# pkusys/Auncel

Hardware: AMD Instinct MI355X
Metric: queries/sec @ recall@10>=0.95, SIFT-10M d=128 IVF4096, 1/2/4/8 GPU (higher is better)
Workload: dtype u8

## Files before the change

### auncel_amd/csrc/ivf_plan.hip

```cpp
#include "ivf_dev.h"

#include <stdlib.h>

namespace amdivf {

__device__ __forceinline__ void plan_begin(const PlanArgs& a, uint32_t tid, uint32_t nthreads) {
    if (tid < 16 && a.history) a.history[tid] = a.counters[tid];
    if (tid == 0 && a.first_plan) {
        a.bytes[0] = 0.0;
        a.acc64[0] = a.acc64[1] = 0ull;
        if (a.min_bytes) a.min_bytes[0] = 0.0;
        if (a.min_bytes_thr) a.min_bytes_thr[0] = 0.0;
    }
    if (a.first_plan && a.round_unfinished)
        for (uint32_t r = tid; r < PLAN_MAX_ROUNDS * 8; r += nthreads) a.round_unfinished[r] = 0;
}
__device__ __forceinline__ void plan_counts_query(const PlanArgs& a, uint32_t i, uint32_t lane) {
    const bool have = i < a.nq;
    uint32_t cnt = 0, pad = 0, more = 0;
    unsigned long long need = 0;
    const unsigned long long ra = a.row_align - 1;
    if (have && !a.done[i]) {
        const uint32_t stage = a.stage[i];
        unsigned long long target = (unsigned long long)stage + a.round_len;
        const unsigned long long np = a.my_nprobe ? a.my_nprobe[a.id_offset + i] : 0ull;
        if (a.tune) {
            const unsigned long long safe = (unsigned long long)((float)(stage + 1) * a.multipler);
            const unsigned long long g = (unsigned long long)((double)stage * a.grow);
            target = safe > g ? safe : g;
            const unsigned long long inc = stage == 0 ? a.first_round : a.min_inc;
            if (target < (unsigned long long)stage + inc) target = (unsigned long long)stage + inc;
        }
        if (np != 0) target = np > (unsigned long long)stage + 1 ? np : (unsigned long long)stage + 1;
        bool last = false;
        if (a.budget_ms) {
            target = (unsigned long long)stage + a.first_round;
            if (stage > 0) {
                const float per = a.elapsed_ms / (float)stage, room = 0.95f * a.budget_ms[a.id_offset + i] - a.elapsed_ms;
                const float fit = room > 0.f ? floorf(room / fmaxf(per, 1e-9f)) : 0.f;
                const unsigned long long cap = stage > a.first_round ? stage : a.first_round;
                unsigned long long len = fit >= (float)a.total_nprobe ? a.total_nprobe : (unsigned long long)fit;
                if (len < 1) len = 1;
                last = len <= cap;
                target = (unsigned long long)stage + (last ? len : cap);
            }
        }
        if (target > a.total_nprobe) target = a.total_nprobe;
        if (a.run_dis && target > stage) {
            const float* dq = a.run_dis + (size_t)i * a.key_stride;
            const int64_t* ka = a.keys + (size_t)i * a.key_stride;
            while (target < a.total_nprobe && dq[target - 1] == dq[target] && ka[target] >= 0) target++;
        }
        if (a.limit && lane == 0) a.limit[i] = last ? (uint32_t)target : a.total_nprobe;
        if (target <= stage) target = stage + 1 < a.total_nprobe ? stage + 1 : a.total_nprobe;
        cnt = (uint32_t)(target - stage);
        const bool ends = target >= a.total_nprobe || last || (a.tune && np != 0);
        more = ends ? 0u : 1u;
        const int64_t* kq = a.keys + (size_t)i * a.key_stride + stage;
        for (uint32_t p = lane; p < cnt; p += 64) {
            const int64_t key = kq[p];
            if (key >= 0 && (unsigned long long)key < a.nlist) {
                const unsigned long long sz = a.list_off[key + 1] - a.list_off[key], psz = (sz + ra) & ~ra;
                need += psz;
                pad += (uint32_t)(psz - sz);
            }
        }
        for (int off = 32; off; off >>= 1) {
            need += __shfl_xor(need, off);
            pad += __shfl_xor(pad, off);
        }
    }
    if (have && lane == 0) {
        a.cnt[i] = cnt;
        a.need[i] = need;
        a.pad[i] = pad | (more << 31);
    }
}
__global__ __launch_bounds__(256) void plan_counts_kernel(PlanArgs a) {
    for (uint32_t l = blockIdx.x * 256 + threadIdx.x; l < 8 * a.nlist; l += gridDim.x * 256) a.xcount[l] = 0;
    if (blockIdx.x == 0) plan_begin(a, threadIdx.x, 256);
    plan_counts_query(a, blockIdx.x * 4 + (threadIdx.x >> 6), threadIdx.x & 63);
}

template <int N> __device__ __forceinline__ void block_scan_1024_n(const uint32_t (&v)[N], uint32_t (&excl)[N], uint32_t (&total)[N],
                                                                    uint32_t (*s_wave)[N]) {
    const int lane = threadIdx.x & 63, w = threadIdx.x >> 6, nw = (int)(blockDim.x >> 6);
    uint32_t incl[N];
#pragma unroll
    for (int k = 0; k < N; k++) incl[k] = v[k];
    for (int off = 1; off < 64; off <<= 1) {
#pragma unroll
        for (int k = 0; k < N; k++) {
            const uint32_t o = (uint32_t)__shfl_up((int)incl[k], off);
            if (lane >= off) incl[k] += o;
        }
    }
    if (lane == 63) {
#pragma unroll
        for (int k = 0; k < N; k++) s_wave[w][k] = incl[k];
    }
    __syncthreads();
    if (w == 0) {
#pragma unroll
        for (int k = 0; k < N; k++) {
            const uint32_t x = lane < nw ? s_wave[lane][k] : 0u;
            uint32_t inc = x;
            for (int off = 1; off < 16; off <<= 1) {
                const uint32_t o = (uint32_t)__shfl_up((int)inc, off);
                if (lane >= off) inc += o;
            }
            if (lane < nw) s_wave[lane][k] = inc - x;
            if (lane == nw - 1) s_wave[16][k] = inc;
        }
    }
    __syncthreads();
#pragma unroll
    for (int k = 0; k < N; k++) {
        excl[k] = s_wave[w][k] + incl[k] - v[k];
        total[k] = s_wave[16][k];
    }
    __syncthreads();
}

__device__ __forceinline__ void plan_prefix_body(const PlanArgs& a) {
    __shared__ uint32_t cut;
    const uint32_t t = threadIdx.x;
    if (t == 0) cut = 0xffffffffu;
    const uint32_t nt = blockDim.x;
    const uint32_t per = (a.nq + nt - 1) / nt, q0 = t * per < a.nq ? t * per : a.nq, q1 = q0 + per < a.nq ? q0 + per : a.nq;
    unsigned long long my_need = 0;
    uint32_t my_cnt = 0, my_act = 0;
    for (uint32_t i = q0; i < q1; i++) {
        const uint32_t c = a.cnt[i];
        my_cnt += c;
        my_act += c ? 1u : 0u;
        my_need += a.need[i];
    }
    unsigned long long tot_need;
    uint32_t ecnt, eact;
    unsigned long long eneed;
    {
        __shared__ uint32_t s_w4[17][4];
        const uint32_t v4[4] = {(uint32_t)(my_need & 0xfffffu), (uint32_t)(my_need >> 20), my_cnt, my_act};
        uint32_t e4[4], t4[4];
        block_scan_1024_n<4>(v4, e4, t4, s_w4);
        eneed = (unsigned long long)e4[0] + ((unsigned long long)e4[1] << 20);
        tot_need = (unsigned long long)t4[0] + ((unsigned long long)t4[1] << 20);
        ecnt = e4[2];
        eact = e4[3];
    }
    for (uint32_t i = q0; i < q1; i++) {
        const uint32_t c = a.cnt[i];
        const unsigned long long nd = a.need[i];
        const bool fits = (eneed + nd <= a.dist_budget && ecnt + c <= a.seg_cap) || eact == 0;
        if (c && !fits) atomicMin(&cut, i);
        a.seg_begin[i] = ecnt;
        a.dist_base[i] = eneed;
        if (c) a.qsel[eact] = i;
        eneed += nd;
        ecnt += c;
        eact += c ? 1u : 0u;
    }
    __syncthreads();
    uint32_t nact = 0, nseg = 0, nmore = 0, ndef = 0;
    unsigned long long ndist = 0;
    __shared__ uint32_t s_nact, s_nseg, s_more, s_def;
    __shared__ unsigned long long s_ndist;
    if (t == 0) {
        s_nact = 0;
        s_nseg = 0;
        s_more = 0;
        s_def = 0;
        s_ndist = 0;
    }
    __syncthreads();
    for (uint32_t i = t; i < a.nq; i += nt) {
        uint32_t c = a.cnt[i];
        const uint32_t pm = a.pad[i], pad = pm & 0x7fffffffu;
        if (pm >> 31) a.pad[i] = pad;
        if (i >= cut && c) {
            a.cnt[i] = c = 0;
            ndef++;
        }
        if (c) {
            nact++;
            nseg += c;
            ndist += a.need[i] - pad;
            nmore += pm >> 31;
        }
    }
    atomicAdd(&s_nact, nact);
    atomicAdd(&s_nseg, nseg);
    atomicAdd(&s_more, nmore);
    atomicAdd(&s_def, ndef);
    atomicAdd(&s_ndist, ndist);
    __syncthreads();
    if (t == 0) {
        a.counters[0] = s_nact;
        a.counters[1] = s_nseg;
        if (a.cl_cursor)
            for (int x = 0; x < 8; x++) a.cl_cursor[32 * x] = 0;
        a.counters[10] = s_more + s_def;
        a.counters[11] = s_def;
        a.counters[7] = (uint32_t)(s_ndist >> 20);
        a.counters[12] = (uint32_t)((tot_need + (1u << 20) - 1) >> 20);
        a.bytes[0] += (double)s_ndist * (double)a.d * 4.0;
        if (a.min_bytes) a.min_bytes[0] += a.dense_round ? (double)s_ndist * 4.0 : (double)s_ndist / 8.0;
        if (a.min_bytes_thr && !a.dense_round) a.min_bytes_thr[0] += (double)s_ndist / 8.0;
    }
}
__global__ __launch_bounds__(1024) void plan_prefix_kernel(PlanArgs a) { plan_prefix_body(a); }

__device__ __forceinline__ void plan_segments_query(const PlanArgs& a, uint32_t i, uint32_t c, uint32_t lane) {
    const uint32_t stage = a.stage[i];
    const uint32_t xcc = xcc_id();
    const int64_t* kq = a.keys + (size_t)i * a.key_stride + stage;
    unsigned long long cur = a.dist_base[i];
    const unsigned long long ra = a.row_align - 1;
    const uint32_t sb = a.seg_begin[i];
    for (uint32_t p0 = 0; p0 < c; p0 += 64) {
        const uint32_t p = p0 + lane;
        int64_t key = -1;
        unsigned long long psz = 0;
        if (p < c) {
            key = kq[p];
            if (key >= 0 && (unsigned long long)key < a.nlist) {
                const unsigned long long sz = a.list_off[key + 1] - a.list_off[key];
                if (sz) {
                    a.seg_slot[sb + p] = (xcc << 28) | xcd_local_add(&a.xcount[xcc * a.nlist + (uint32_t)key], 1u);
                    psz = (sz + ra) & ~ra;
                }
            }
        }
        unsigned long long incl = psz;
        for (int off = 1; off < 64; off <<= 1) {
            const unsigned long long o = __shfl_up(incl, off);
            if ((int)lane >= off) incl += o;
        }
        if (p < c) {
            a.seg_list[sb + p] = (int32_t)key;
            a.seg_off[sb + p] = cur + incl - psz;
        }
        cur += __shfl(incl, 63);
    }
}
__global__ __launch_bounds__(256) void plan_segments_kernel(PlanArgs a) {
    const uint32_t i = blockIdx.x * 4 + (threadIdx.x >> 6);
    const uint32_t c = i < a.nq ? a.cnt[i] : 0u;
    if (c) plan_segments_query(a, i, c, threadIdx.x & 63);
}


__device__ __forceinline__ void plan_lists_body(const PlanArgs& a) {
    __shared__ uint32_t s_w[17][6];
    const uint32_t t = threadIdx.x;
    auto values = [&](uint32_t l, uint32_t c, uint32_t (&v)[6]) {
#pragma unroll
        for (int k = 0; k < 6; k++) v[k] = 0;
        if (!c) return;
        const unsigned long long sz = a.list_off[l + 1] - a.list_off[l];
        v[0] = c;
        v[1] = (c + SCAN_RQ - 1) / SCAN_RQ;
        if (a.mfma_chunk) {
            v[5] = ((c + a.mfma_qblock - 1) / a.mfma_qblock) * (uint32_t)((sz + a.mfma_chunk - 1) / a.mfma_chunk);
            return;
        }
        const uint32_t full = c / a.qblock, rem = c % a.qblock;
        if (full) {
            const uint32_t qg = scan_shape_of(a.qblock);
            const uint32_t tv = scan_tile_vecs(qg);
            v[2 + scan_qg_class(qg)] = full * (uint32_t)((sz + tv - 1) / tv);
        }
        if (rem) {
            const uint32_t qg = scan_shape_of(rem);
            const uint32_t tv = scan_tile_vecs(qg);
            v[2 + scan_qg_class(qg)] += (uint32_t)((sz + tv - 1) / tv);
        }
    };
    auto book = [&](uint32_t l, uint32_t c, unsigned long long& slots, unsigned long long& useful) {
        if (!c) return;
        const unsigned long long sz = a.list_off[l + 1] - a.list_off[l];
        useful += (unsigned long long)c * sz;
        if (a.mfma_chunk) {
            const unsigned long long nvb = (sz + a.mfma_chunk - 1) / a.mfma_chunk, lastv = sz - (nvb - 1) * a.mfma_chunk;
            const unsigned long long vsum = (nvb - 1) * (((unsigned long long)a.mfma_chunk + 63) / 64 * 64) + (lastv + 63) / 64 * 64;
            const unsigned long long nqb = (c + a.mfma_qblock - 1) / a.mfma_qblock, lastq = c - (nqb - 1) * a.mfma_qblock;
            const unsigned long long qsum = (nqb - 1) * (((unsigned long long)a.mfma_qblock + MFMA_QBLOCK - 1) / MFMA_QBLOCK * MFMA_QBLOCK) +
                                            (lastq + MFMA_QBLOCK - 1) / MFMA_QBLOCK * MFMA_QBLOCK;
            slots += qsum * vsum;
            return;
        }
        const uint32_t full = c / a.qblock, rem = c % a.qblock;
        if (full) {
            const uint32_t tv = scan_tile_vecs(scan_shape_of(a.qblock));
            slots += (unsigned long long)full * ((a.qblock + SCAN_RQ - 1) / SCAN_RQ * SCAN_RQ) * ((sz + tv - 1) / tv) * tv;
        }
        if (rem) {
            const uint32_t tv = scan_tile_vecs(scan_shape_of(rem));
            slots += (unsigned long long)((rem + SCAN_RQ - 1) / SCAN_RQ * SCAN_RQ) * ((sz + tv - 1) / tv) * tv;
        }
    };
    const uint32_t nt = blockDim.x;
    const uint32_t per = (a.nlist + nt - 1) / nt, l0 = t * per < a.nlist ? t * per : a.nlist, l1 = l0 + per < a.nlist ? l0 + per : a.nlist;
    uint32_t mine[6] = {0, 0, 0, 0, 0, 0};
    double list_bytes = 0;
    unsigned long long my_slots = 0, my_useful = 0;
    for (uint32_t l = l0; l < l1; l++) {
        uint32_t c = 0;
#pragma unroll
        for (uint32_t x = 0; x < 8; x++) {
            const uint32_t cx = a.xcount[x * a.nlist + l];
            a.xcount[x * a.nlist + l] = c;
            c += cx;
        }
        a.lcount[l] = c;
        book(l, c, my_slots, my_useful);
        uint32_t v[6];
        values(l, c, v);
#pragma unroll
        for (int k = 0; k < 6; k++) mine[k] += v[k];
        if (v[0]) list_bytes += (double)(a.list_off[l + 1] - a.list_off[l]) * (double)a.row_bytes;
    }
    for (int off = 32; off; off >>= 1) {
        my_slots += __shfl_xor(my_slots, off);
        my_useful += __shfl_xor(my_useful, off);
    }
    if ((t & 63) == 0 && my_slots) {
        atomicAdd(&a.acc64[0], my_slots);
        atomicAdd(&a.acc64[1], my_useful);
    }
    if (a.min_bytes && list_bytes > 0) atomicAdd(a.min_bytes, list_bytes);
    if (a.min_bytes_thr && !a.dense_round && list_bytes > 0) atomicAdd(a.min_bytes_thr, list_bytes);
    uint32_t ex[6], tot[6];
    block_scan_1024_n<6>(mine, ex, tot, s_w);
    for (uint32_t l = l0; l < l1; l++) {
        uint32_t v[6];
        values(l, a.lcount[l], v);
        a.lstart[l] = ex[0];
        a.gbase[l] = ex[1];
        a.ibase[0 * a.nlist + l] = ex[2];
        a.ibase[1 * a.nlist + l] = ex[3];
        a.ibase[2 * a.nlist + l] = ex[4];
        a.ibase[3 * a.nlist + l] = ex[5];
#pragma unroll
        for (int k = 0; k < 6; k++) ex[k] += v[k];
    }
    if (t == 0) {
        const bool over = (unsigned long long)tot[2] + tot[3] + tot[4] + tot[5] > (unsigned long long)a.item_cap;
        if (over) {
            atomicMax(a.error, ERR_ITEM_OVERFLOW);
            tot[2] = tot[3] = tot[4] = tot[5] = 0;
        }
        a.counters[2] = tot[0];
        a.counters[3] = tot[1];
        a.counters[4] = tot[2];
        a.counters[5] = tot[3];
        a.counters[8] = tot[4];
        a.counters[9] = tot[5];
    }
}
__global__ __launch_bounds__(1024) void plan_lists_kernel(PlanArgs a) { plan_lists_body(a); }

__device__ __forceinline__ void plan_scatter_query(const PlanArgs& a, uint32_t i, uint32_t lane) {
    if (i >= a.nq) return;
    const uint32_t c = a.cnt[i];
    if (!c) return;
    const uint32_t sb = a.seg_begin[i];
    for (uint32_t p = lane; p < c; p += 64) {
        const int32_t key = a.seg_list[sb + p];
        if (key < 0 || (uint32_t)key >= a.nlist) continue;
        if (a.list_off[key + 1] == a.list_off[key]) continue;
        const uint32_t ss = a.seg_slot[sb + p];
        const uint32_t pos = a.lstart[key] + a.xcount[(ss >> 28) * a.nlist + (uint32_t)key] + (ss & 0x0fffffffu);
        a.pair_query[pos] = a.slot_base + i;
        a.pair_out[pos] = a.seg_off[sb + p];
    }
}

__device__ inline void items_of_list(const PlanArgs& a, uint32_t l, uint32_t c) {
    const uint32_t p0 = a.lstart[l], g0 = a.gbase[l];
    for (uint32_t o = 0, g = 0; o < c; o += SCAN_RQ, g++) {
        a.group_p0[g0 + g] = p0 + o;
        a.group_cnt[g0 + g] = c - o < (uint32_t)SCAN_RQ ? c - o : (uint32_t)SCAN_RQ;
    }
    const uint32_t n1 = a.counters[4], n2 = a.counters[5], n4 = a.counters[8];
    uint32_t cur[4] = {a.ibase[l], n1 + a.ibase[a.nlist + l], n1 + n2 + a.ibase[2 * a.nlist + l],
                       n1 + n2 + n4 + a.ibase[3 * a.nlist + l]};
    const uint32_t sz = (uint32_t)(a.list_off[l + 1] - a.list_off[l]);
    const uint64_t vb0 = a.list_off[l];
    const uint64_t lb0 = a.lane_block_off ? a.lane_block_off[l] : 0ull;
    if (a.mfma_chunk) {
        uint32_t ni = cur[3];
        const uint64_t b0 = a.block_off[l];
        const uint32_t nvb = (sz + a.mfma_chunk - 1) / a.mfma_chunk, nqb = (c + a.mfma_qblock - 1) / a.mfma_qblock;
        for (uint32_t o = 0; o < nvb * nqb; o++) {
            const uint32_t vb = (a.item_order ? o % nvb : o / nqb) * a.mfma_chunk, qb = (a.item_order ? o / nvb : o % nqb) * a.mfma_qblock;
            {
                ScanItem it;
                it.vec_base = b0 + vb / MFMA_BLOCK;
                it.nvec = sz - vb < a.mfma_chunk ? sz - vb : a.mfma_chunk;
                it.vec_off = vb;
                it.pair_begin = p0 + qb;
                it.npair = c - qb < a.mfma_qblock ? c - qb : a.mfma_qblock;
                it.qg = 0;
                it.qgroup = (uint32_t)(vb0 + vb);
                if (ni < a.item_cap) a.items[ni] = it;
                ni++;
            }
        }
        return;
    }
    for (uint32_t qb = 0; qb < c; qb += a.qblock) {
        const uint32_t nq_blk = c - qb < a.qblock ? c - qb : a.qblock;
        const uint32_t qg = scan_shape_of(nq_blk);
        const uint32_t tv = scan_tile_vecs(qg);
        uint32_t& ni = cur[scan_qg_class(qg)];
        for (uint32_t vb = 0; vb < sz; vb += tv) {
            ScanItem it;
            it.vec_base = scan_vec_base(vb0 + vb, lb0, vb);
            it.nvec = sz - vb < tv ? sz - vb : tv;
            it.vec_off = vb;
            it.pair_begin = p0 + qb;
            it.npair = nq_blk;
            it.qg = qg;
            it.qgroup = g0 + qb / SCAN_RQ;
            if (ni < a.item_cap) a.items[ni] = it;
            ni++;
        }
    }
}


__device__ __forceinline__ void plan_items_lists(const PlanArgs& a, uint32_t l) {
    const uint32_t c = l < a.nlist ? a.lcount[l] : 0u;
    if (c) items_of_list(a, l, c);
}

__device__ inline void items_of_list_wave(const PlanArgs& a, uint32_t l, uint32_t c, uint32_t lane) {
    const uint32_t p0 = a.lstart[l], g0 = a.gbase[l];
    for (uint32_t g = lane; g * SCAN_RQ < c; g += 64) {
        const uint32_t o = g * SCAN_RQ;
        a.group_p0[g0 + g] = p0 + o;
        a.group_cnt[g0 + g] = c - o < (uint32_t)SCAN_RQ ? c - o : (uint32_t)SCAN_RQ;
    }
    const uint32_t n1 = a.counters[4], n2 = a.counters[5], n4 = a.counters[8];
    const uint32_t cur[4] = {a.ibase[l], n1 + a.ibase[a.nlist + l], n1 + n2 + a.ibase[2 * a.nlist + l],
                             n1 + n2 + n4 + a.ibase[3 * a.nlist + l]};
    const uint32_t sz = (uint32_t)(a.list_off[l + 1] - a.list_off[l]);
    const uint64_t vb0 = a.list_off[l];
    const uint64_t lb0 = a.lane_block_off ? a.lane_block_off[l] : 0ull;
    if (a.mfma_chunk) {
        const uint64_t b0 = a.block_off[l];
        const uint32_t nvb = (sz + a.mfma_chunk - 1) / a.mfma_chunk, nqb = (c + a.mfma_qblock - 1) / a.mfma_qblock;
        for (uint32_t o = lane; o < nvb * nqb; o += 64) {
            const uint32_t vb = (a.item_order ? o % nvb : o / nqb) * a.mfma_chunk, qb = (a.item_order ? o / nvb : o % nqb) * a.mfma_qblock;
            ScanItem it;
            it.vec_base = b0 + vb / MFMA_BLOCK;
            it.nvec = sz - vb < a.mfma_chunk ? sz - vb : a.mfma_chunk;
            it.vec_off = vb;
            it.pair_begin = p0 + qb;
            it.npair = c - qb < a.mfma_qblock ? c - qb : a.mfma_qblock;
            it.qg = 0;
            it.qgroup = (uint32_t)(vb0 + vb);
            if (cur[3] + o < a.item_cap) a.items[cur[3] + o] = it;
        }
        return;
    }
    const uint32_t full = c / a.qblock, rem = c % a.qblock;
    const uint32_t qg_f = scan_shape_of(a.qblock), tv_f = scan_tile_vecs(qg_f), nt_f = (sz + tv_f - 1) / tv_f;
    const int cls_f = scan_qg_class(qg_f);
    for (uint32_t o = lane; o < full * nt_f; o += 64) {
        const uint32_t qb = (o / nt_f) * a.qblock, vb = (o % nt_f) * tv_f;
        ScanItem it;
        it.vec_base = scan_vec_base(vb0 + vb, lb0, vb);
        it.nvec = sz - vb < tv_f ? sz - vb : tv_f;
        it.vec_off = vb;
        it.pair_begin = p0 + qb;
        it.npair = a.qblock;
        it.qg = qg_f;
        it.qgroup = g0 + qb / SCAN_RQ;
        if (cur[cls_f] + o < a.item_cap) a.items[cur[cls_f] + o] = it;
    }
    if (rem) {
        const uint32_t qg_r = scan_shape_of(rem), tv_r = scan_tile_vecs(qg_r), nt_r = (sz + tv_r - 1) / tv_r;
        const int cls_r = scan_qg_class(qg_r);
        const uint32_t base = cur[cls_r] + (cls_r == cls_f ? full * nt_f : 0u), qb = full * a.qblock;
        for (uint32_t o = lane; o < nt_r; o += 64) {
            const uint32_t vb = o * tv_r;
            ScanItem it;
            it.vec_base = scan_vec_base(vb0 + vb, lb0, vb);
            it.nvec = sz - vb < tv_r ? sz - vb : tv_r;
            it.vec_off = vb;
            it.pair_begin = p0 + qb;
            it.npair = rem;
            it.qg = qg_r;
            it.qgroup = g0 + qb / SCAN_RQ;
            if (base + o < a.item_cap) a.items[base + o] = it;
        }
    }
}

__global__ __launch_bounds__(256) void plan_scatter_items_kernel(PlanArgs a, uint32_t gq) {
    if (blockIdx.x < gq) {
        plan_scatter_query(a, blockIdx.x * 4 + (threadIdx.x >> 6), threadIdx.x & 63);
        return;
    }
    const uint32_t l = (blockIdx.x - gq) * 4 + (threadIdx.x >> 6);
    const uint32_t c = l < a.nlist ? a.lcount[l] : 0u;
    if (c) items_of_list_wave(a, l, c, threadIdx.x & 63);
}

constexpr uint32_t PLAN_SMALL_NQ = 32;
__global__ __launch_bounds__(1024) void plan_small_kernel(PlanArgs a) {
    const uint32_t tid = threadIdx.x, lane = tid & 63, wave = tid >> 6;
    for (uint32_t l = tid; l < 8 * a.nlist; l += 1024) a.xcount[l] = 0;
    plan_begin(a, tid, 1024);
    __syncthreads();
    for (uint32_t i = wave; i < a.nq; i += 16) plan_counts_query(a, i, lane);
    __syncthreads();
    plan_prefix_body(a);
    __syncthreads();
    for (uint32_t i = wave; i < a.nq; i += 16) {
        const uint32_t c = a.cnt[i];
        if (c) plan_segments_query(a, i, c, lane);
    }
    __syncthreads();
    plan_lists_body(a);
    __syncthreads();
    for (uint32_t i = wave; i < a.nq; i += 16) plan_scatter_query(a, i, lane);
    for (uint32_t l0 = 0; l0 < a.nlist; l0 += 1024) plan_items_lists(a, l0 + tid);
}

__global__ __launch_bounds__(64) void plan_one_kernel(PlanArgs a) {
    const uint32_t lane = threadIdx.x;
    plan_begin(a, lane, 64);
    __syncthreads();
    plan_counts_query(a, 0, lane);
    __syncthreads();
    const uint32_t c = a.cnt[0];
    const unsigned long long nd = a.need[0];
    const uint32_t pm = a.pad[0], pad = pm & 0x7fffffffu;
    const unsigned long long ndist = c ? nd - pad : 0ull;
    if (lane == 0) {
        if (pm >> 31) a.pad[0] = pad;
        a.seg_begin[0] = 0;
        a.dist_base[0] = 0;
        if (c) a.qsel[0] = 0;
        a.counters[0] = c ? 1u : 0u;
        a.counters[1] = c;
        a.counters[10] = c ? pm >> 31 : 0u;
        a.counters[11] = 0;
        a.counters[7] = (uint32_t)(ndist >> 20);
        a.counters[12] = (uint32_t)((nd + (1u << 20) - 1) >> 20);
        a.bytes[0] += (double)ndist * (double)a.d * 4.0;
        if (a.min_bytes) a.min_bytes[0] += a.dense_round ? (double)ndist * 4.0 : (double)ndist / 8.0;
        if (a.min_bytes_thr && !a.dense_round) a.min_bytes_thr[0] += (double)ndist / 8.0;
    }
    const uint32_t stage = a.stage[0];
    const int64_t* kq = a.keys + stage;
    const unsigned long long ra = a.row_align - 1;
    const unsigned long long lt = lane == 0 ? 0ull : (~0ull >> (64 - lane));
    unsigned long long cur = 0, slots = 0, useful = 0;
    uint32_t np = 0, ni = 0;
    double list_bytes = 0;
    const uint32_t tv1 = scan_tile_vecs(1);
    for (uint32_t p0 = 0; p0 < c; p0 += 64) {
        const uint32_t p = p0 + lane;
        int64_t key = -1;
        uint32_t sz = 0;
        if (p < c) {
            key = kq[p];
            if (key >= 0 && (unsigned long long)key < a.nlist) sz = (uint32_t)(a.list_off[key + 1] - a.list_off[key]);
        }
        const bool valid = sz != 0;
        const unsigned long long psz = valid ? ((unsigned long long)sz + ra) & ~ra : 0ull;
        unsigned long long incl = psz;
        for (int off = 1; off < 64; off <<= 1) {
            const unsigned long long o = __shfl_up(incl, off);
            if ((int)lane >= off) incl += o;
        }
        const unsigned long long my_off = cur + incl - psz;
        if (p < c) {
            a.seg_list[p] = (int32_t)key;
            a.seg_off[p] = my_off;
        }
        cur += __shfl(incl, 63);
        const unsigned long long vm = __ballot(valid);
        const uint32_t pidx = np + (uint32_t)__builtin_popcountll(vm & lt);
        const uint32_t tile = a.mfma_chunk ? a.mfma_chunk : tv1;
        const uint32_t n_it = valid ? (sz + tile - 1) / tile : 0u;
        uint32_t iincl = n_it;
        for (int off = 1; off < 64; off <<= 1) {
            const uint32_t o = (uint32_t)__shfl_up((int)iincl, off);
            if ((int)lane >= off) iincl += o;
        }
        const uint32_t ibase = ni + iincl - n_it;
        if (valid) {
            a.pair_query[pidx] = a.slot_base;
            a.pair_out[pidx] = my_off;
            a.group_p0[pidx] = pidx;
            a.group_cnt[pidx] = 1;
            const uint64_t vb0 = a.list_off[key];
            const uint64_t b0 = a.mfma_chunk ? a.block_off[key] : 0ull;
            for (uint32_t o = 0; o < n_it; o++) {
                const uint32_t vb = o * tile;
                ScanItem it;
                it.vec_base = a.mfma_chunk ? b0 + vb / MFMA_BLOCK : scan_vec_base(vb0 + vb, a.lane_block_off ? a.lane_block_off[key] : 0ull, vb);
                it.nvec = sz - vb < tile ? sz - vb : tile;
                it.vec_off = vb;
                it.pair_begin = pidx;
                it.npair = 1;
                it.qg = a.mfma_chunk ? 0u : 1u;
                it.qgroup = a.mfma_chunk ? (uint32_t)(vb0 + vb) : pidx;
                if (ibase + o < a.item_cap) a.items[ibase + o] = it;
                slots += a.mfma_chunk ? (unsigned long long)MFMA_QBLOCK * (((it.nvec + 63) / 64) * 64) : (unsigned long long)SCAN_RQ * tile;
            }
            useful += sz;
            list_bytes += (double)sz * (double)a.row_bytes;
        }
        np += (uint32_t)__builtin_popcountll(vm);
        ni += (uint32_t)__shfl((int)iincl, 63);
    }
    for (int off = 32; off; off >>= 1) {
        slots += __shfl_xor(slots, off);
        useful += __shfl_xor(useful, off);
        list_bytes += __shfl_xor(list_bytes, off);
    }
    if (lane == 0) {
        const bool over = ni > a.item_cap;
        if (over) atomicMax(a.error, ERR_ITEM_OVERFLOW);
        const uint32_t nit = over ? 0u : ni;
        a.counters[2] = np;
        a.counters[3] = np;
        a.counters[4] = a.mfma_chunk ? 0u : nit;
        a.counters[5] = 0;
        a.counters[8] = 0;
        a.counters[9] = a.mfma_chunk ? nit : 0u;
        if (a.min_bytes && list_bytes > 0) a.min_bytes[0] += list_bytes;
        if (a.min_bytes_thr && !a.dense_round && list_bytes > 0) a.min_bytes_thr[0] += list_bytes;
        if (slots) {
            a.acc64[0] += slots;
            a.acc64[1] += useful;
        }
    }
}

void launch_plan(const PlanArgs& a, hipStream_t s) {
    if (a.nq == 0) return;
    static const bool no_one = getenv("AUNCEL_AMD_NO_PLAN_ONE") != nullptr;
    if (a.nq == 1 && !no_one) {
        LAUNCH(plan_one_kernel, dim3(1), dim3(64), 0, s, a);
        return;
    }
    if (a.nq <= PLAN_SMALL_NQ && a.nlist <= 65536) {
        LAUNCH(plan_small_kernel, dim3(1), dim3(1024), 0, s, a);
        return;
    }
    const unsigned gq = (a.nq + 3) / 4 , gl = (a.nlist + 3) / 4 ;
    static const unsigned plan_threads = [] {
        const char* e = getenv("AUNCEL_AMD_PLAN_THREADS");
        const int v = e ? atoi(e) : 1024;
        return (unsigned)(v >= 64 && v <= 1024 && v % 64 == 0 ? v : 1024);
    }();
    LAUNCH(plan_counts_kernel, dim3(gq), dim3(256), 0, s, a);
    LAUNCH(plan_prefix_kernel, dim3(1), dim3(plan_threads), 0, s, a);
    LAUNCH(plan_segments_kernel, dim3(gq), dim3(256), 0, s, a);
    LAUNCH(plan_lists_kernel, dim3(1), dim3(plan_threads), 0, s, a);
    LAUNCH(plan_scatter_items_kernel, dim3(gq + gl), dim3(256), 0, s, a, (uint32_t)gq);
}


__global__ void xcd_check_kernel(uint32_t* counters, uint32_t nkeys, uint32_t* slot, uint32_t* xcc_of, uint32_t n) {
    const uint32_t i = blockIdx.x * blockDim.x + threadIdx.x;
    if (i >= n) return;
    const uint32_t key = (i * 2654435761u) % nkeys;
    uint32_t x;
    asm volatile("s_getreg_b32 %0, hwreg(HW_REG_XCC_ID)" : "=s"(x));
    x &= 0xfu;
    slot[i] = x < 8 ? xcd_local_add(&counters[x * nkeys + key], 1u) : 0u;
    xcc_of[i] = x;
}
void launch_xcd_check(uint32_t* counters, uint32_t nkeys, uint32_t* slot, uint32_t* xcc_of, uint32_t n, hipStream_t s) {
    LAUNCH(xcd_check_kernel, dim3((n + 255) / 256), dim3(256), 0, s, counters, nkeys, slot, xcc_of, n);
}

}
```

Before: 2.973 million.

## Shrink single-block plan kernels to 256 threads with batched vector loads and DPP scans

```diff
diff --git a/auncel_amd/csrc/ivf_plan.hip b/auncel_amd/csrc/ivf_plan.hip
--- a/auncel_amd/csrc/ivf_plan.hip
+++ b/auncel_amd/csrc/ivf_plan.hip
@@ -82,19 +82,22 @@
     plan_counts_query(a, blockIdx.x * 4 + (threadIdx.x >> 6), threadIdx.x & 63);
 }
 
-template <int N> __device__ __forceinline__ void block_scan_1024_n(const uint32_t (&v)[N], uint32_t (&excl)[N], uint32_t (&total)[N],
-                                                                    uint32_t (*s_wave)[N]) {
+
+__device__ __forceinline__ uint32_t wave_incl_sum(uint32_t x) {
+    x += (uint32_t)__builtin_amdgcn_update_dpp(0, (int)x, 0x111, 0xf, 0xf, false);
+    x += (uint32_t)__builtin_amdgcn_update_dpp(0, (int)x, 0x112, 0xf, 0xf, false);
+    x += (uint32_t)__builtin_amdgcn_update_dpp(0, (int)x, 0x114, 0xf, 0xf, false);
+    x += (uint32_t)__builtin_amdgcn_update_dpp(0, (int)x, 0x118, 0xf, 0xf, false);
+    x += (uint32_t)__builtin_amdgcn_update_dpp(0, (int)x, 0x142, 0xa, 0xf, false);
+    x += (uint32_t)__builtin_amdgcn_update_dpp(0, (int)x, 0x143, 0xc, 0xf, false);
+    return x;
+}
+template <int N> __device__ __forceinline__ void block_scan_n(const uint32_t (&v)[N], uint32_t (&excl)[N], uint32_t (&total)[N],
+                                                               uint32_t (*s_wave)[N]) {
     const int lane = threadIdx.x & 63, w = threadIdx.x >> 6, nw = (int)(blockDim.x >> 6);
     uint32_t incl[N];
 #pragma unroll
-    for (int k = 0; k < N; k++) incl[k] = v[k];
-    for (int off = 1; off < 64; off <<= 1) {
-#pragma unroll
-        for (int k = 0; k < N; k++) {
-            const uint32_t o = (uint32_t)__shfl_up((int)incl[k], off);
-            if (lane >= off) incl[k] += o;
-        }
-    }
+    for (int k = 0; k < N; k++) incl[k] = wave_incl_sum(v[k]);
     if (lane == 63) {
 #pragma unroll
         for (int k = 0; k < N; k++) s_wave[w][k] = incl[k];
@@ -104,11 +107,7 @@
 #pragma unroll
         for (int k = 0; k < N; k++) {
             const uint32_t x = lane < nw ? s_wave[lane][k] : 0u;
-            uint32_t inc = x;
-            for (int off = 1; off < 16; off <<= 1) {
-                const uint32_t o = (uint32_t)__shfl_up((int)inc, off);
-                if (lane >= off) inc += o;
-            }
+            const uint32_t inc = wave_incl_sum(x);
             if (lane < nw) s_wave[lane][k] = inc - x;
             if (lane == nw - 1) s_wave[16][k] = inc;
         }
@@ -122,6 +121,8 @@
     __syncthreads();
 }
 
+constexpr uint32_t PLAN_BATCH = 4;
+constexpr uint32_t PLAN_THREADS = 256;
 __device__ __forceinline__ void plan_prefix_body(const PlanArgs& a) {
     __shared__ uint32_t cut;
     const uint32_t t = threadIdx.x;
@@ -130,11 +131,21 @@
     const uint32_t per = (a.nq + nt - 1) / nt, q0 = t * per < a.nq ? t * per : a.nq, q1 = q0 + per < a.nq ? q0 + per : a.nq;
     unsigned long long my_need = 0;
     uint32_t my_cnt = 0, my_act = 0;
-    for (uint32_t i = q0; i < q1; i++) {
-        const uint32_t c = a.cnt[i];
-        my_cnt += c;
-        my_act += c ? 1u : 0u;
-        my_need += a.need[i];
+    for (uint32_t i0 = q0; i0 < q1; i0 += PLAN_BATCH) {
+        uint32_t c[PLAN_BATCH];
+        unsigned long long nd[PLAN_BATCH];
+#pragma unroll
+        for (uint32_t j = 0; j < PLAN_BATCH; j++) {
+            const bool in = i0 + j < q1;
+            c[j] = in ? a.cnt[i0 + j] : 0u;
+            nd[j] = in ? a.need[i0 + j] : 0ull;
+        }
+#pragma unroll
+        for (uint32_t j = 0; j < PLAN_BATCH; j++) {
+            my_cnt += c[j];
+            my_act += c[j] ? 1u : 0u;
+            my_need += nd[j];
+        }
     }
     unsigned long long tot_need;
     uint32_t ecnt, eact;
@@ -143,23 +154,36 @@
         __shared__ uint32_t s_w4[17][4];
         const uint32_t v4[4] = {(uint32_t)(my_need & 0xfffffu), (uint32_t)(my_need >> 20), my_cnt, my_act};
         uint32_t e4[4], t4[4];
-        block_scan_1024_n<4>(v4, e4, t4, s_w4);
+        block_scan_n<4>(v4, e4, t4, s_w4);
         eneed = (unsigned long long)e4[0] + ((unsigned long long)e4[1] << 20);
         tot_need = (unsigned long long)t4[0] + ((unsigned long long)t4[1] << 20);
         ecnt = e4[2];
         eact = e4[3];
     }
-    for (uint32_t i = q0; i < q1; i++) {
-        const uint32_t c = a.cnt[i];
-        const unsigned long long nd = a.need[i];
-        const bool fits = (eneed + nd <= a.dist_budget && ecnt + c <= a.seg_cap) || eact == 0;
-        if (c && !fits) atomicMin(&cut, i);
-        a.seg_begin[i] = ecnt;
-        a.dist_base[i] = eneed;
-        if (c) a.qsel[eact] = i;
-        eneed += nd;
-        ecnt += c;
-        eact += c ? 1u : 0u;
+    for (uint32_t i0 = q0; i0 < q1; i0 += PLAN_BATCH) {
+        uint32_t cb[PLAN_BATCH];
+        unsigned long long ndb[PLAN_BATCH];
+#pragma unroll
+        for (uint32_t j = 0; j < PLAN_BATCH; j++) {
+            const bool in = i0 + j < q1;
+            cb[j] = in ? a.cnt[i0 + j] : 0u;
+            ndb[j] = in ? a.need[i0 + j] : 0ull;
+        }
+#pragma unroll
+        for (uint32_t j = 0; j < PLAN_BATCH; j++) {
+            const uint32_t i = i0 + j;
+            if (i >= q1) break;
+            const uint32_t c = cb[j];
+            const unsigned long long nd = ndb[j];
+            const bool fits = (eneed + nd <= a.dist_budget && ecnt + c <= a.seg_cap) || eact == 0;
+            if (c && !fits) atomicMin(&cut, i);
+            a.seg_begin[i] = ecnt;
+            a.dist_base[i] = eneed;
+            if (c) a.qsel[eact] = i;
+            eneed += nd;
+            ecnt += c;
+            eact += c ? 1u : 0u;
+        }
     }
     __syncthreads();
     uint32_t nact = 0, nseg = 0, nmore = 0, ndef = 0;
@@ -174,26 +198,50 @@
         s_ndist = 0;
     }
     __syncthreads();
-    for (uint32_t i = t; i < a.nq; i += nt) {
-        uint32_t c = a.cnt[i];
-        const uint32_t pm = a.pad[i], pad = pm & 0x7fffffffu;
-        if (pm >> 31) a.pad[i] = pad;
-        if (i >= cut && c) {
-            a.cnt[i] = c = 0;
-            ndef++;
-        }
-        if (c) {
-            nact++;
-            nseg += c;
-            ndist += a.need[i] - pad;
-            nmore += pm >> 31;
-        }
-    }
-    atomicAdd(&s_nact, nact);
-    atomicAdd(&s_nseg, nseg);
-    atomicAdd(&s_more, nmore);
-    atomicAdd(&s_def, ndef);
-    atomicAdd(&s_ndist, ndist);
+    const uint32_t cut_at = cut;
+    for (uint32_t i0 = t; i0 < a.nq; i0 += PLAN_BATCH * nt) {
+        uint32_t cb[PLAN_BATCH], pmb[PLAN_BATCH];
+        unsigned long long ndb[PLAN_BATCH];
+#pragma unroll
+        for (uint32_t j = 0; j < PLAN_BATCH; j++) {
+            const uint32_t i = i0 + j * nt;
+            const bool in = i < a.nq;
+            cb[j] = in ? a.cnt[i] : 0u;
+            pmb[j] = in ? a.pad[i] : 0u;
+            ndb[j] = in ? a.need[i] : 0ull;
+        }
+#pragma unroll
+        for (uint32_t j = 0; j < PLAN_BATCH; j++) {
+            const uint32_t i = i0 + j * nt;
+            uint32_t c = cb[j];
+            const uint32_t pm = pmb[j], pad = pm & 0x7fffffffu;
+            if (pm >> 31) a.pad[i] = pad;
+            if (i >= cut_at && c) {
+                a.cnt[i] = c = 0;
+                ndef++;
+            }
+            if (c) {
+                nact++;
+                nseg += c;
+                ndist += ndb[j] - pad;
+                nmore += pm >> 31;
+            }
+        }
+    }
+    for (int off = 32; off; off >>= 1) {
+        nact += __shfl_xor(nact, off);
+        nseg += __shfl_xor(nseg, off);
+        nmore += __shfl_xor(nmore, off);
+        ndef += __shfl_xor(ndef, off);
+        ndist += __shfl_xor(ndist, off);
+    }
+    if ((t & 63) == 0) {
+        atomicAdd(&s_nact, nact);
+        atomicAdd(&s_nseg, nseg);
+        atomicAdd(&s_more, nmore);
+        atomicAdd(&s_def, ndef);
+        atomicAdd(&s_ndist, ndist);
+    }
     __syncthreads();
     if (t == 0) {
         a.counters[0] = s_nact;
@@ -209,7 +257,7 @@
         if (a.min_bytes_thr && !a.dense_round) a.min_bytes_thr[0] += (double)s_ndist / 8.0;
     }
 }
-__global__ __launch_bounds__(1024) void plan_prefix_kernel(PlanArgs a) { plan_prefix_body(a); }
+__global__ __launch_bounds__(PLAN_THREADS) void plan_prefix_kernel(PlanArgs a) { plan_prefix_body(a); }
 
 __device__ __forceinline__ void plan_segments_query(const PlanArgs& a, uint32_t i, uint32_t c, uint32_t lane) {
     const uint32_t stage = a.stage[i];
@@ -254,11 +302,10 @@
 __device__ __forceinline__ void plan_lists_body(const PlanArgs& a) {
     __shared__ uint32_t s_w[17][6];
     const uint32_t t = threadIdx.x;
-    auto values = [&](uint32_t l, uint32_t c, uint32_t (&v)[6]) {
+    auto values = [&](unsigned long long sz, uint32_t c, uint32_t (&v)[6]) {
 #pragma unroll
         for (int k = 0; k < 6; k++) v[k] = 0;
         if (!c) return;
-        const unsigned long long sz = a.list_off[l + 1] - a.list_off[l];
         v[0] = c;
         v[1] = (c + SCAN_RQ - 1) / SCAN_RQ;
         if (a.mfma_chunk) {
@@ -277,9 +324,8 @@
             v[2 + scan_qg_class(qg)] += (uint32_t)((sz + tv - 1) / tv);
         }
     };
-    auto book = [&](uint32_t l, uint32_t c, unsigned long long& slots, unsigned long long& useful) {
+    auto book = [&](unsigned long long sz, uint32_t c, unsigned long long& slots, unsigned long long& useful) {
         if (!c) return;
-        const unsigned long long sz = a.list_off[l + 1] - a.list_off[l];
         useful += (unsigned long long)c * sz;
         if (a.mfma_chunk) {
             const unsigned long long nvb = (sz + a.mfma_chunk - 1) / a.mfma_chunk, lastv = sz - (nvb - 1) * a.mfma_chunk;
@@ -301,25 +347,68 @@
         }
     };
     const uint32_t nt = blockDim.x;
-    const uint32_t per = (a.nlist + nt - 1) / nt, l0 = t * per < a.nlist ? t * per : a.nlist, l1 = l0 + per < a.nlist ? l0 + per : a.nlist;
+    const uint32_t per = ((a.nlist + nt - 1) / nt + PLAN_BATCH - 1) / PLAN_BATCH * PLAN_BATCH;
+    const uint32_t l0 = t * per < a.nlist ? t * per : a.nlist, l1 = l0 + per < a.nlist ? l0 + per : a.nlist;
+    static_assert(PLAN_BATCH == 4, "a batch is one uint4");
+    const bool vec = (a.nlist & 3u) == 0 && (((uintptr_t)a.xcount | (uintptr_t)a.lcount | (uintptr_t)a.lstart | (uintptr_t)a.gbase | (uintptr_t)a.ibase |
+                                              (uintptr_t)a.list_off) & 15u) == 0;
+    auto bounds = [&](uint32_t lb, uint64_t (&lo)[PLAN_BATCH + 1]) {
+        if (vec) {
+            const ulonglong2 p = *reinterpret_cast<const ulonglong2*>(a.list_off + lb), q = *reinterpret_cast<const ulonglong2*>(a.list_off + lb + 2);
+            lo[0] = p.x, lo[1] = p.y, lo[2] = q.x, lo[3] = q.y, lo[4] = a.list_off[lb + 4];
+        } else {
+#pragma unroll
+            for (uint32_t j = 0; j <= PLAN_BATCH; j++) lo[j] = a.list_off[lb + j <= l1 ? lb + j : l1];
+        }
+    };
+    auto put4 = [&](uint32_t* arr, uint32_t lb, const uint32_t (&w)[PLAN_BATCH]) {
+        if (vec) {
+            *reinterpret_cast<uint4*>(arr + lb) = make_uint4(w[0], w[1], w[2], w[3]);
+        } else {
+#pragma unroll
+            for (uint32_t j = 0; j < PLAN_BATCH; j++)
+                if (lb + j < l1) arr[lb + j] = w[j];
+        }
+    };
+    auto get4 = [&](const uint32_t* arr, uint32_t lb, uint32_t (&w)[PLAN_BATCH]) {
+        if (vec) {
+            const uint4 q = *reinterpret_cast<const uint4*>(arr + lb);
+            w[0] = q.x, w[1] = q.y, w[2] = q.z, w[3] = q.w;
+        } else {
+#pragma unroll
+            for (uint32_t j = 0; j < PLAN_BATCH; j++) w[j] = lb + j < l1 ? arr[lb + j] : 0u;
+        }
+    };
     uint32_t mine[6] = {0, 0, 0, 0, 0, 0};
     double list_bytes = 0;
     unsigned long long my_slots = 0, my_useful = 0;
-    for (uint32_t l = l0; l < l1; l++) {
-        uint32_t c = 0;
-#pragma unroll
-        for (uint32_t x = 0; x < 8; x++) {
-            const uint32_t cx = a.xcount[x * a.nlist + l];
-            a.xcount[x * a.nlist + l] = c;
-            c += cx;
-        }
-        a.lcount[l] = c;
-        book(l, c, my_slots, my_useful);
-        uint32_t v[6];
-        values(l, c, v);
-#pragma unroll
-        for (int k = 0; k < 6; k++) mine[k] += v[k];
-        if (v[0]) list_bytes += (double)(a.list_off[l + 1] - a.list_off[l]) * (double)a.row_bytes;
+    for (uint32_t lb = l0; lb < l1; lb += PLAN_BATCH) {
+        uint32_t cx[8][PLAN_BATCH], lc[PLAN_BATCH];
+        uint64_t lo[PLAN_BATCH + 1];
+#pragma unroll
+        for (uint32_t x = 0; x < 8; x++) get4(a.xcount + x * a.nlist, lb, cx[x]);
+        bounds(lb, lo);
+#pragma unroll
+        for (uint32_t j = 0; j < PLAN_BATCH; j++) {
+            uint32_t c = 0;
+#pragma unroll
+            for (uint32_t x = 0; x < 8; x++) {
+                const uint32_t n = cx[x][j];
+                cx[x][j] = c;
+                c += n;
+            }
+            lc[j] = c;
+            const unsigned long long sz = lo[j + 1] - lo[j];
+            book(sz, c, my_slots, my_useful);
+            uint32_t v[6];
+            values(sz, c, v);
+#pragma unroll
+            for (int k = 0; k < 6; k++) mine[k] += v[k];
+            if (v[0]) list_bytes += (double)sz * (double)a.row_bytes;
+        }
+#pragma unroll
+        for (uint32_t x = 0; x < 8; x++) put4(a.xcount + x * a.nlist, lb, cx[x]);
+        put4(a.lcount, lb, lc);
     }
     for (int off = 32; off; off >>= 1) {
         my_slots += __shfl_xor(my_slots, off);
@@ -332,18 +421,26 @@
     if (a.min_bytes && list_bytes > 0) atomicAdd(a.min_bytes, list_bytes);
     if (a.min_bytes_thr && !a.dense_round && list_bytes > 0) atomicAdd(a.min_bytes_thr, list_bytes);
     uint32_t ex[6], tot[6];
-    block_scan_1024_n<6>(mine, ex, tot, s_w);
-    for (uint32_t l = l0; l < l1; l++) {
-        uint32_t v[6];
-        values(l, a.lcount[l], v);
-        a.lstart[l] = ex[0];
-        a.gbase[l] = ex[1];
-        a.ibase[0 * a.nlist + l] = ex[2];
-        a.ibase[1 * a.nlist + l] = ex[3];
-        a.ibase[2 * a.nlist + l] = ex[4];
-        a.ibase[3 * a.nlist + l] = ex[5];
-#pragma unroll
-        for (int k = 0; k < 6; k++) ex[k] += v[k];
+    block_scan_n<6>(mine, ex, tot, s_w);
+    for (uint32_t lb = l0; lb < l1; lb += PLAN_BATCH) {
+        uint32_t cb[PLAN_BATCH], o[6][PLAN_BATCH];
+        uint64_t lo[PLAN_BATCH + 1];
+        get4(a.lcount, lb, cb);
+        bounds(lb, lo);
+#pragma unroll
+        for (uint32_t j = 0; j < PLAN_BATCH; j++) {
+            uint32_t v[6];
+            values(lo[j + 1] - lo[j], cb[j], v);
+#pragma unroll
+            for (int k = 0; k < 6; k++) {
+                o[k][j] = ex[k];
+                ex[k] += v[k];
+            }
+        }
+        put4(a.lstart, lb, o[0]);
+        put4(a.gbase, lb, o[1]);
+#pragma unroll
+        for (uint32_t k = 0; k < 4; k++) put4(a.ibase + k * a.nlist, lb, o[2 + k]);
     }
     if (t == 0) {
         const bool over = (unsigned long long)tot[2] + tot[3] + tot[4] + tot[5] > (unsigned long long)a.item_cap;
@@ -359,7 +456,7 @@
         a.counters[9] = tot[5];
     }
 }
-__global__ __launch_bounds__(1024) void plan_lists_kernel(PlanArgs a) { plan_lists_body(a); }
+__global__ __launch_bounds__(PLAN_THREADS) void plan_lists_kernel(PlanArgs a) { plan_lists_body(a); }
 
 __device__ __forceinline__ void plan_scatter_query(const PlanArgs& a, uint32_t i, uint32_t lane) {
     if (i >= a.nq) return;
@@ -657,15 +754,10 @@
         return;
     }
     const unsigned gq = (a.nq + 3) / 4 , gl = (a.nlist + 3) / 4 ;
-    static const unsigned plan_threads = [] {
-        const char* e = getenv("AUNCEL_AMD_PLAN_THREADS");
-        const int v = e ? atoi(e) : 1024;
-        return (unsigned)(v >= 64 && v <= 1024 && v % 64 == 0 ? v : 1024);
-    }();
     LAUNCH(plan_counts_kernel, dim3(gq), dim3(256), 0, s, a);
-    LAUNCH(plan_prefix_kernel, dim3(1), dim3(plan_threads), 0, s, a);
+    LAUNCH(plan_prefix_kernel, dim3(1), dim3(PLAN_THREADS), 0, s, a);
     LAUNCH(plan_segments_kernel, dim3(gq), dim3(256), 0, s, a);
-    LAUNCH(plan_lists_kernel, dim3(1), dim3(plan_threads), 0, s, a);
+    LAUNCH(plan_lists_kernel, dim3(1), dim3(PLAN_THREADS), 0, s, a);
     LAUNCH(plan_scatter_items_kernel, dim3(gq + gl), dim3(256), 0, s, a, (uint32_t)gq);
 }
 
```

Result: no change. 2.950 million (-0.7%).
